# cmhungsteve/TA3N

Measured on AMD Instinct MI355X. Metric: src+tgt videos/sec per train step, UCF->HMDB_full 5-seg TA3N, higher is better.
Workload: dtype bf16

## Files before the change

ta3n_amd/csrc/ta3n_gemm_kernel.h:

```cpp
#pragma once
#include <hip/hip_runtime.h>
#include <cstdlib>
#include <cstring>

#include <type_traits>

#include "ta3n_kernels.h"

using namespace ta3n;

namespace {

typedef float f32x16 __attribute__((ext_vector_type(16)));
typedef __attribute__((address_space(3))) void lds_void_t;

constexpr int BKC = 64;

__device__ __forceinline__ float4 zero4() { return make_float4(0.f, 0.f, 0.f, 0.f); }

__device__ __forceinline__ void glds16(const float *gsrc, unsigned lds_byte_addr) {
    unsigned keep;
    lds_byte_addr = __builtin_amdgcn_readfirstlane(lds_byte_addr);
    asm volatile("s_mov_b32 %0, m0\n\ts_mov_b32 m0, %2\n\ts_nop 0\n\tglobal_load_lds_dwordx4 %1, off\n\ts_mov_b32 m0, %0"
                 : "=&s"(keep) : "v"(gsrc), "s"(lds_byte_addr) : "memory");
// ... 37 lines not shown
    asm volatile("s_mov_b32 %0, m0\n\ts_mov_b32 m0, %2\n\ts_nop 0\n\tglobal_load_lds_dword %1, off\n\ts_mov_b32 m0, %0"
                 : "=&s"(keep) : "v"(gsrc), "s"(lds_byte_addr) : "memory");
}

template <int R, int NW>
__device__ __attribute__((noinline)) void issue_slow(const float *__restrict__ origin, int ld, int kmajor, int r0, int rvalid, int k0,
                                                     int krem, unsigned lds_addr, int wave, int lane, const float *__restrict__ zeros) {
#pragma unroll 1
    for (int q = wave; q < R; q += NW) {
        const float *src;
        if (!kmajor) {
            const int k = 4 * ((lane >> 2) ^ (q & 15)) + (lane & 3);
            src = (r0 + q < rvalid && k < krem) ? origin + (size_t)(r0 + q) * ld + k0 + k : zeros;
        } else {
            constexpr int KPP = 64 / R;
            const int k = q * KPP + lane / R;
            const int r = r0 + lane % R;
            src = (r < rvalid && k < krem) ? origin + (size_t)(k0 + k) * ld + r : zeros;
        }
        glds4(src, lds_addr + q * 256);
    }
}

constexpr int K_NEVER = 1 << 28;

template <int R, int NW, bool TW = false, bool PAIR = false, bool HS = false>
struct OperandStream {
    static constexpr int NP = HS ? R / 8 / NW : R / 4 / NW;
    static_assert(HS ? (R / 8) % NW == 0 && TW && !PAIR : (R / 4) % NW == 0, "pieces must divide over the waves");
    const float *p[NP];
    int kofs[NP];
    int step;
    const float *origin;
    int ld, kmajor, r0, rvalid;
    bool vec;

    __device__ __forceinline__ void setup(const float *__restrict__ origin_, int ld_, int kmajor_, int klen, int r0_, int rvalid_,
                                          int wave, int lane, int pair_delta = 0) {
        origin = origin_; ld = ld_; kmajor = kmajor_; r0 = r0_; rvalid = rvalid_;
        if constexpr (TW && PAIR) {
            vec = true;
            const int ldf = ld_ >> 1;
            step = kmajor_ ? 64 * ldf : BKC / 2;
#pragma unroll
            for (int i = 0; i < NP; ++i) {
                const int q = wave + NW * i;
// ... 17 lines not shown
            vec = true;
            const int ldf = ld_ >> 1;
            step = kmajor_ ? 64 * ldf : BKC / 2;
#pragma unroll
            for (int i = 0; i < NP; ++i) {
                const int q = wave + NW * i;
                if (!kmajor_) {
                    const int row = q * 8 + (lane >> 3);
                    const int slot = (lane & 7) ^ ((row >> 1) & 7);
                    p[i] = origin_ + (size_t)(r0_ + row) * ldf + 4 * slot;
                    kofs[i] = (r0_ + row < rvalid_) ? 8 * slot : K_NEVER;
                } else {
                    constexpr int LPR = R / 8, KPP = 64 / LPR;
                    const int k = q * KPP + lane / LPR;
                    const int chunk = (lane % LPR) ^ (R == 64 ? ((k >> 1) & 1) << 2 : R == 128 ? (k & 3) << 2 : 0);
                    const int r = r0_ + chunk * 8;
                    p[i] = origin_ + (size_t)k * ldf + (r >> 1);
                    kofs[i] = (r < rvalid_) ? k : K_NEVER;
                }
            }
            return;
        }
        if constexpr (TW) {
            vec = true;
            const int ldf = ld_ >> 1;
            step = kmajor_ ? 128 * ldf : BKC;
#pragma unroll
            for (int i = 0; i < NP; ++i) {
                const int q = wave + NW * i;
                if (!kmajor_) {
                    const int row = q * 4 + (lane >> 4);
                    const int slot = (lane & 15) ^ (row & 15);
                    p[i] = origin_ + (size_t)(r0_ + row) * ldf + 4 * slot;
                    kofs[i] = (r0_ + row < rvalid_) ? 8 * slot : K_NEVER;
                } else {
                    constexpr int LPR = R / 8, KPP = 64 / LPR;
                    const int k = q * KPP + lane / LPR;
                    const int chunk = (lane % LPR) ^ (R == 64 ? ((k >> 1) & 1) << 2 : R == 128 ? (k & 3) << 2 : 0);
                    const int r = r0_ + chunk * 8;
                    p[i] = origin_ + (size_t)k * ldf + (r >> 1);
                    kofs[i] = (r < rvalid_) ? k : K_NEVER;
                }
            }
            return;
        }
        const int off_bits = (int)(reinterpret_cast<uintptr_t>(origin_) >> 2);
        vec = kmajor_ ? (((off_bits | ld_ | r0_ | rvalid_) & 3) == 0) : (((off_bits | ld_ | klen) & 3) == 0);
// ... 6 lines not shown
                const int row = q * 4 + (lane >> 4);
                const int k = 4 * ((lane & 15) ^ (row & 15));
                p[i] = origin_ + (size_t)(r0_ + row) * ld_ + k;
                kofs[i] = (r0_ + row < rvalid_) ? k : K_NEVER;
            } else {
                constexpr int LPR = R / 4, KPP = 64 / LPR;
                const int k = q * KPP + lane / LPR;
                const int r = r0_ + (lane % LPR) * 4;
                p[i] = origin_ + (size_t)k * ld_ + r;
                kofs[i] = (r < rvalid_) ? k : K_NEVER;
            }
        }
    }

    __device__ __forceinline__ void issue(int k0, int krem, unsigned lds_addr, int wave, int lane, const float *__restrict__ zeros) {
        if (vec) {
            const float *src[NP];
#pragma unroll
            for (int i = 0; i < NP; ++i) {
                src[i] = kofs[i] < krem ? p[i] : zeros;
                p[i] += step;
            }
            glds16_batch<NP>(src, lds_addr + wave * 1024, NW * 1024);
        } else {
            issue_slow<R, NW>(origin, ld, kmajor, r0, rvalid, k0, krem, lds_addr, wave, lane, zeros);
        }
    }
};

typedef short s16x4 __attribute__((ext_vector_type(4)));
typedef float f32x4 __attribute__((ext_vector_type(4)));
typedef __bf16 bf16x2 __attribute__((ext_vector_type(2)));
typedef __bf16 bf16x8 __attribute__((ext_vector_type(8)));
typedef float f32x2 __attribute__((ext_vector_type(2)));
typedef unsigned u32x2 __attribute__((ext_vector_type(2)));
typedef unsigned u32x4 __attribute__((ext_vector_type(4)));


template <int BM, int BN, int WK, bool AKM, bool BKM, bool FULL, bool RS, int BF, int RM = 1, int RN = 1>
__device__ __forceinline__ void compute_stage(f32x16 (&accs)[RM][RN], float (&rss)[RM], const float *__restrict__ sa,
                                              const float *__restrict__ sb, int ra, int rb, int wk, int lh, int krem) {
    constexpr bool HS = BF == 5;
    constexpr int GPW = (HS ? 8 : 16) / WK;
    constexpr int NQ = GPW / 2;
    constexpr int ROWF = HS ? BKC / 2 : BKC;
    static_assert(GPW >= 2, "the K split leaves every wave a pair of k groups");
// ... 1078 lines not shown
```

ta3n_amd/csrc/ta3n_heads.hip:

```cpp
#include <hip/hip_runtime.h>

#include <mutex>

#include "../../include/ta3n_hip.h"
#include "ta3n_kernels.h"

using namespace ta3n;

namespace {

typedef float f32x4 __attribute__((ext_vector_type(4)));


constexpr int NBH = 256;
constexpr int RPW = HEADS_RPW;
constexpr int WROW = 68;
constexpr int TROW = 260;

template <int VPW>
struct Lds {
    static_assert(VPW == 1 || VPW == 2, "1 or 2 videos per workgroup");
    static constexpr int W = 0;
    static constexpr int VD = W + NBH * WROW;
    static constexpr int HV = VD + VPW * NBH;
    static constexpr int GHV = HV + VPW * NBH;
    static constexpr int GVT = GHV + VPW * NBH;
    static constexpr int GY = GVT + VPW * NBH;
    static constexpr int PR = GY + VPW * 64;
    static constexpr int GPV = PR + VPW * 128;
    static constexpr int Y = GPV + 8;
    static constexpr int FPART = Y + VPW * 64;
    static constexpr int VPART = FPART + 16 * NBH;
    static constexpr int LOSS = VPART + 4 * NBH;
    static constexpr int TOTAL = LOSS + 32;
    static constexpr int WPV = 4 / VPW;
};
static_assert(64 * TROW <= NBH * WROW, "backward tile / classifier staging must fit in the weight tile");
constexpr int S_LOSS_MIN = Lds<1>::LOSS;

#ifdef TA3N_HEADS_TIMING
#define STAMP(i) do { if ((int)blockIdx.x == g.n_frm_wg + 100 && threadIdx.x == 0) { reinterpret_cast<unsigned long long *>(ptrs.ws + g.o_gattn)[i] = __builtin_amdgcn_s_memtime(); } } while (0)
#else
#define STAMP(i) do { } while (0)
#endif

__device__ __forceinline__ bool video_valid(int Bs, int valid_source, int valid_target, int b) {
    return b < Bs ? (b < valid_source) : (b - Bs < valid_target);
}

struct StepScalars {
    int valid_source, valid_target;
    float inv_n_cls, inv_n_rel, inv_n_vid, inv_n_frm, inv_n_ent, gamma, beta1, p_drop_v;
    uint32_t seed_v;
};
__device__ __forceinline__ StepScalars step_scalars(const Hyper *__restrict__ hy) {
    StepScalars h;
    h.valid_source = hy->valid_source; h.valid_target = hy->valid_target;
    h.inv_n_cls = hy->inv_n_cls; h.inv_n_rel = hy->inv_n_rel; h.inv_n_vid = hy->inv_n_vid; h.inv_n_frm = hy->inv_n_frm;
    h.inv_n_ent = hy->inv_n_ent; h.gamma = hy->gamma; h.beta1 = hy->beta[1]; h.p_drop_v = hy->p_drop_v; h.seed_v = hy->seed_v;
    return h;
}

__device__ __forceinline__ void write_loss_part(float *smem, float *ws, int o_loss_part, int wg, float gamma, int S_LOSS) {
    const int tid = threadIdx.x;
    __syncthreads();
    float v = 0.f;
    if (tid < 8) v = (smem[S_LOSS + tid] + smem[S_LOSS + 8 + tid]) + (smem[S_LOSS + 16 + tid] + smem[S_LOSS + 24 + tid]);
    __syncthreads();
// ... 5 lines not shown
    }
}

template <int VPW, bool PIPE>
__device__ __forceinline__ void video_wg(const Geom g, const Ptrs ptrs, float *smem) {
    using L = Lds<VPW>;
    constexpr int S_W = L::W, S_VD = L::VD, S_HV = L::HV, S_GHV = L::GHV, S_GVT = L::GVT, S_GY = L::GY, S_PR = L::PR, S_GPV = L::GPV, S_Y = L::Y,
                  S_FPART = L::FPART, S_VPART = L::VPART, S_LOSS = L::LOSS, WPV = L::WPV;
    float *__restrict__ ws = ptrs.ws;
    const float *__restrict__ wsr = ptrs.ws;
    const float *__restrict__ P = ptrs.p;
    const Hyper *__restrict__ hy = reinterpret_cast<const Hyper *>(ptrs.ws + g.o_hyper);
    const int *__restrict__ tf = reinterpret_cast<const int *>(ptrs.ws + g.o_tuple_first);
    const int *__restrict__ labels = reinterpret_cast<const int *>(ptrs.ws + g.o_labels);
    const int tid = threadIdx.x, lane = tid & 63, wv = tid >> 6;
    const int NR = g.n_rel, NT = g.n_tuples, C = g.C;
    const int b0 = ((int)blockIdx.x - g.n_frm_wg) * VPW;
    const int nv = min(VPW, g.B - b0);
    const int vloc = wv / WPV, sub = wv % WPV;
    const int b = b0 + vloc;
    const bool have = vloc < nv;
    const bool lead = sub == 0;
    const bool attn_on = (g.flags & TA3N_FLAG_TRANS_ATTN) != 0;
    const bool train = hy->train != 0;
    const StepScalars hs = step_scalars(hy);
    const float inv_keep_v = hyper_scale(hy, SK_INV_KEEP_V);
    const bool drop_v = train && hs.p_drop_v > 0.f;
    const float *__restrict__ Wdv = P + g.p_Wdv;
    const float *__restrict__ Wcv = P + g.p_Wcv;
    float l_cls = 0.f, l_rel = 0.f, l_vid = 0.f, l_ent = 0.f;

    const int tfv = lane <= NR ? tf[lane] : 0;
    struct RelIn { float hr[4], w0[4], w1[4], zr[3][4], b0, b1; int nt; };
    auto load_rel = [&](int j, RelIn &o) {
        const float *__restrict__ W2f = P + g.p_W2_0 + (size_t)j * g.p_W2_stride;
        const float *__restrict__ hrf = wsr + g.o_Hr + ((size_t)b * NR + j) * NBH;
        const int ju = __builtin_amdgcn_readfirstlane(j);
        const int t_lo = __builtin_amdgcn_readlane(tfv, ju);
        const int t_hi = __builtin_amdgcn_readlane(tfv, ju + 1);
        o.nt = t_hi - t_lo;
#pragma unroll
        for (int q = 0; q < 4; ++q) { o.hr[q] = hrf[q * 64 + lane]; o.w0[q] = W2f[q * 64 + lane]; o.w1[q] = W2f[NBH + q * 64 + lane]; }
#pragma unroll
        for (int tt = 0; tt < 3; ++tt) {
            const bool on = tt < o.nt;
#pragma unroll
// ... 35 lines not shown
#pragma unroll 1
            for (int j = sub; j < NR; j += WPV) {
                RelIn rel_nxt = rel_cur;
                if (PIPE && j + WPV < NR) load_rel(j + WPV, rel_nxt);
                float d0 = 0.f, d1 = 0.f;
                float r[4] = {0.f, 0.f, 0.f, 0.f};
#pragma unroll
                for (int q = 0; q < 4; ++q) {
                    d0 = fmaf(rel_cur.hr[q], rel_cur.w0[q], d0);
                    d1 = fmaf(rel_cur.hr[q], rel_cur.w1[q], d1);
                }
#pragma unroll
                for (int tt = 0; tt < 3; ++tt)
#pragma unroll
                    for (int q = 0; q < 4; ++q) r[q] += rel_cur.zr[tt][q];
                d0 = wave_allreduce_sum(d0) + rel_cur.b0;
                d1 = wave_allreduce_sum(d1) + rel_cur.b1;
                if (PIPE) rel_cur = rel_nxt;
                float w = 0.f;
                if (attn_on) w = 1.f - soft2(d0, d1).H;
#pragma unroll
                for (int q = 0; q < 4; ++q) {
                    ws[g.o_R + ((size_t)b * NR + j) * NBH + q * 64 + lane] = r[q];
                    vacc[q] += attn_on ? (w + 1.f) * r[q] : r[q];
                }
                if (lane == 0) {
                    ws[g.o_Pr + ((size_t)b * NR + j) * 2 + 0] = d0;
                    ws[g.o_Pr + ((size_t)b * NR + j) * 2 + 1] = d1;
                    ws[g.o_attn + (size_t)b * NR + j] = attn_on ? w : r[0];
                    smem[S_PR + (vloc * 64 + j) * 2 + 0] = d0;
                    smem[S_PR + (vloc * 64 + j) * 2 + 1] = d1;
                }
            }
        }
#pragma unroll
        for (int q = 0; q < 4; ++q) smem[S_VPART + wv * NBH + q * 64 + lane] = vacc[q];
    }
    __syncthreads();
#pragma unroll
    for (int v = 0; v < VPW; ++v) {
        float val = 0.f;
#pragma unroll
        for (int s_ = 0; s_ < WPV; ++s_) val += smem[S_VPART + (v * WPV + s_) * NBH + tid];
        float vd = val;
        if (drop_v) vd = val * keep_mask(hs.seed_v, (uint32_t)((b0 + v) * NBH + tid), hs.p_drop_v) * inv_keep_v;
        if (v < nv) {
            ws[g.o_V + (size_t)(b0 + v) * NBH + tid] = val;
            ws[g.o_Vd + (size_t)(b0 + v) * NBH + tid] = vd;
        }
        smem[S_VD + v * NBH + tid] = v < nv ? vd : 0.f;
    }
    STAMP(1);
#pragma unroll
    for (int i = 0; i < 16; ++i) {
        const int f = i * 256 + tid;
        if (f < C * 64) *reinterpret_cast<f32x4 *>(&smem[S_W + (f >> 6) * TROW + (f & 63) * 4]) = cw[i];
    }
    __syncthreads();

    STAMP(2);
    {
        const int c = tid >> 2, part = tid & 3;
#pragma unroll
        for (int v = 0; v < VPW; ++v) {
            float acc = 0.f;
            if (c < C) {
                const float *wr = &smem[S_W + c * TROW + part * 64];
                const float *vd = &smem[S_VD + v * NBH + part * 64];
#pragma unroll
                for (int k4 = 0; k4 < 64; k4 += 4) {
                    const float4 w4 = *reinterpret_cast<const float4 *>(wr + k4);
// ... 19 lines not shown
        const int n = srow + 16 * c16;
#pragma unroll
        for (int v = 0; v < VPW; ++v) {
            f32x4 xk[4];
#pragma unroll
            for (int kc = 0; kc < 4; ++kc) xk[kc] = *reinterpret_cast<const f32x4 *>(&smem[S_VD + v * NBH + kc * 64 + sk4]);
            float hv = 0.f;
#pragma unroll
            for (int i = 0; i < 16; ++i) {
                float p = 0.f;
#pragma unroll
                for (int kc = 0; kc < 4; ++kc) {
                    const f32x4 w4 = wreg[kc * 16 + i];
                    p = fmaf(w4.x, xk[kc].x, p); p = fmaf(w4.y, xk[kc].y, p); p = fmaf(w4.z, xk[kc].z, p); p = fmaf(w4.w, xk[kc].w, p);
                }
                p += dpp_move<0xB1, 0xF>(0.f, p);
                p += dpp_move<0x4E, 0xF>(0.f, p);
                p += dpp_move<0x141, 0xF>(0.f, p);
                p += dpp_move<0x140, 0xF>(0.f, p);
                if (c16 == i) hv = p;
            }
            const float h = fmaxf(hv + bdv_n, 0.f);
            smem[S_HV + v * NBH + n] = h;
            if (v < nv) ws[g.o_Hv + (size_t)(b0 + v) * NBH + n] = h;
        }
    }
    __syncthreads();

    STAMP(4);
    {
        float d0 = 0.f, d1 = 0.f;
#pragma unroll
        for (int q = 0; q < 4; ++q) {
            const float h = smem[S_HV + vloc * NBH + q * 64 + lane];
            d0 = fmaf(h, wc0[q], d0);
            d1 = fmaf(h, wc1[q], d1);
        }
        d0 = wave_allreduce_sum(d0) + bcdv0;
        d1 = wave_allreduce_sum(d1) + bcdv1;
        const float m = wave_allreduce_max(y);
        const float e = lane < C ? expf(y - m) : 0.f;
        const float ls = logf(wave_allreduce_sum(e));
        const float lp = lane < C ? y - m - ls : 0.f;
        const float pr = lane < C ? expf(lp) : 0.f;
        const float Hc = wave_allreduce_sum(-pr * lp);
        float gy = 0.f, g0 = 0.f, g1 = 0.f;
        if (have && lead) {
// ... 3 lines not shown
            const Soft2 s = soft2(d0, d1);
            const bool ent_on = (g.flags & TA3N_FLAG_ATTN_ENTROPY) && valid;
            const float ce = hs.gamma * hs.inv_n_ent;
            if (cls_on) {
                gy = (pr - (lane == label ? 1.f : 0.f)) * hs.inv_n_cls;
                if (lane == label) l_cls = -lp * hs.inv_n_cls;
            }
            if (ent_on) {
                gy += ce * (1.f + s.H) * (-pr * (lp + Hc));
                if (lane == 0) l_ent = (1.f + s.H) * Hc * hs.inv_n_ent;
            }
            if (lane >= C) gy = 0.f;
            if ((g.flags & TA3N_FLAG_ADV_VIDEO) && valid) {
                const int d = is_src ? 0 : 1;
                if (lane == 0) l_vid = -(d ? s.lp1 : s.lp0) * hs.inv_n_vid;
                g0 = (s.p0 - (d == 0 ? 1.f : 0.f)) * hs.inv_n_vid;
                g1 = (s.p1 - (d == 1 ? 1.f : 0.f)) * hs.inv_n_vid;
            }
            if (ent_on) {
                g0 += ce * Hc * (-s.p0 * (s.lp0 + s.H));
                g1 += ce * Hc * (-s.p1 * (s.lp1 + s.H));
            }
            if (lane < C) ws[g.o_gY + (size_t)b * C + lane] = gy;
            if (lane == 0) {
                ws[g.o_Pv + (size_t)b * 2] = d0; ws[g.o_Pv + (size_t)b * 2 + 1] = d1;
                ws[g.o_gPv + (size_t)b * 2] = g0; ws[g.o_gPv + (size_t)b * 2 + 1] = g1;
            }
        }
        if (lead) {
            smem[S_GY + vloc * 64 + lane] = gy;
            if (lane == 0) { smem[S_GPV + vloc * 2] = g0; smem[S_GPV + vloc * 2 + 1] = g1; }
        }
        l_cls = wave_allreduce_sum(l_cls);
    }
    __syncthreads();

    STAMP(5);
#pragma unroll
    for (int v = 0; v < VPW; ++v) {
        const float gh = smem[S_HV + v * NBH + tid] > 0.f ? smem[S_GPV + v * 2] * wct0 + smem[S_GPV + v * 2 + 1] * wct1 : 0.f;
        smem[S_GHV + v * NBH + tid] = gh;
        if (v < nv) ws[g.o_gHv + (size_t)(b0 + v) * NBH + tid] = gh;
    }
    __syncthreads();

    struct RelBack { float w20[4], w21[4], hrv[4], rv[4]; };
    auto load_back = [&](int j, RelBack &o) {
        const size_t bj = (size_t)b * NR + j;
        const float *__restrict__ W2 = P + g.p_W2_0 + (size_t)j * g.p_W2_stride;
#pragma unroll
        for (int q = 0; q < 4; ++q) {
            const int c = q * 64 + lane;
            o.w20[q] = W2[c]; o.w21[q] = W2[NBH + c];
            o.hrv[q] = wsr[g.o_Hr + bj * NBH + c];
            o.rv[q] = ws[g.o_R + bj * NBH + c];
        }
    };
    RelBack back_cur;
#pragma unroll
    for (int q = 0; q < 4; ++q) back_cur.w20[q] = back_cur.w21[q] = back_cur.hrv[q] = back_cur.rv[q] = 0.f;
    if (PIPE && have && sub < NR) load_back(sub, back_cur);

#pragma unroll
    for (int v = 0; v < VPW; ++v) {
        float gh[16];
// ... 42 lines not shown
#pragma unroll
            for (int q = 0; q < 4; ++q) { w20[q] = back_cur.w20[q]; w21[q] = back_cur.w21[q]; hrv[q] = back_cur.hrv[q]; rv[q] = back_cur.rv[q]; }
            if (PIPE) back_cur = back_nxt;
            const float z0 = smem[S_PR + (vloc * 64 + j) * 2], z1 = smem[S_PR + (vloc * 64 + j) * 2 + 1];
            const Soft2 s = soft2(z0, z1);
            float g0 = 0.f, g1 = 0.f;
            if (adv_rel) {
                const int d = is_src ? 0 : 1;
                if (lane == 0) l_rel += -(d ? s.lp1 : s.lp0) * hs.inv_n_rel;
                g0 = (s.p0 - (d == 0 ? 1.f : 0.f)) * hs.inv_n_rel;
                g1 = (s.p1 - (d == 1 ? 1.f : 0.f)) * hs.inv_n_rel;
            }
            if (lane == 0) { ws[g.o_gPr + bj * 2] = g0; ws[g.o_gPr + bj * 2 + 1] = g1; }
            float w1 = 1.f;
            if (attn_on) {
                float dot = 0.f;
#pragma unroll
                for (int q = 0; q < 4; ++q) dot = fmaf(rv[q], gv[q], dot);
                dot = wave_allreduce_sum(dot);
                g0 += dot * s.p0 * (s.lp0 + s.H);
                g1 += dot * s.p1 * (s.lp1 + s.H);
                w1 = 1.f + (1.f - s.H);
            }
            if (lane == 0) { ws[g.o_gPrT + bj * 2] = g0; ws[g.o_gPrT + bj * 2 + 1] = g1; }
#pragma unroll
            for (int q = 0; q < 4; ++q) {
                const int c = q * 64 + lane;
                ws[g.o_gRa + bj * NBH + c] = w1 * gv[q];
                ws[g.o_gHr + bj * NBH + c] = hrv[q] > 0.f ? g0 * w20[q] + g1 * w21[q] : 0.f;
            }
        }
    }
    {
        auto lane0 = [](float x) { return __builtin_bit_cast(float, __builtin_amdgcn_readlane(__builtin_bit_cast(int, x), 0)); };
        const float lr = lane0(l_rel), lv = lane0(l_vid), le = lane0(l_ent);
        if (lane < 8) {
            float v = 0.f;
            if (lane == 1) v = l_cls;
            if (lane == 2) v = lr;
            if (lane == 3) v = lv;
            if (lane == 5) v = le;
            smem[S_LOSS + wv * 8 + lane] = v;
        }
    }
    STAMP(7);
    write_loss_part(smem, ws, g.o_loss_part, (int)blockIdx.x - g.n_frm_wg, hs.gamma, S_LOSS);
    STAMP(8);
}

template <int FQ>
__device__ __forceinline__ void frame_wg(const Geom g, const Ptrs ptrs, float *smem, int wg) {
    float *__restrict__ ws = ptrs.ws;
// ... 148 lines not shown
```

ta3n_amd/csrc/ta3n_plan.cpp:

```cpp
#include "ta3n_plan.h"
#include "ta3n_kernels.h"

#include <algorithm>
#include <cstdlib>
#include <cstring>
#include <sstream>

using namespace ta3n;

int64_t ta3n_plan::poff(const std::string &name) const {
    for (const auto &p : params)
        if (p.name == name) return p.off;
    return -1;
}
int64_t ta3n_plan::woff(const std::string &name) const {
    for (const auto &r : regions)
        if (r.name == name) return r.off;
    return -1;
}

namespace {

int64_t align_up(int64_t v, int64_t a) { return (v + a - 1) / a * a; }

// ... 548 lines not shown
        for (int i = ph.task_begin; i < ph.task_begin + ph.task_count; ++i) {
            const Task &t = p.tasks[i];
            if (t.seg_count == 0) continue;
            if (t.c_base == BASE_WS) produced.push_back({t.c_off, t.c_off + (int64_t)(t.m_valid - 1) * t.c_ld + t.n_valid});
            for (int f = 0; f < t.fan_count; ++f)
                produced.push_back({t.fan_out_off[f], t.fan_out_off[f] + (int64_t)(t.m_valid - 1) * t.fan_ld + t.n_valid});
        }
    }
    std::vector<Span> read16;
    for (Phase &ph : p.phases) {
        if (!in_family(ph.group) || ph.kind != PH_GEMM) continue;
        bool ok = true;
        std::vector<Span> reads;
        std::vector<char> seen(p.segs.size(), 0);
        for (int i = ph.task_begin; i < ph.task_begin + ph.task_count && ok; ++i) {
            const Task &t = p.tasks[i];
            for (int k = t.seg_begin; k < t.seg_begin + t.seg_count && ok; ++k) {
                if (seen[k]) continue;
                seen[k] = 1;
                const Seg &sg = p.segs[k];
                const int a_rows = sg.pad[0] > 0 ? sg.pad[0] : t.m_valid, b_rows = t.n_valid;
                auto side_ok = [&](int base, int off, int ld, int kmajor, int rows) {
                    if (base == BASE_G) return false;
                    if (((off | ld) & 7) != 0) return false;
                    if ((kmajor ? rows : sg.klen) & 7) return false;
                    if (base == BASE_WS) {
                        const Span rd = kmajor ? Span{off, off + (int64_t)(sg.klen - 1) * ld + rows}
                                               : Span{off, off + (int64_t)(rows - 1) * ld + sg.klen};
                        bool covered = false;
                        for (auto &pr : produced) covered = covered || overlaps(rd, pr);
                        if (!covered) return false;
                        reads.push_back(rd);
                    }
                    return true;
                };
                ok = side_ok(sg.a_base, sg.a_off, sg.a_ld, sg.a_kmajor, a_rows) &&
                     side_ok(sg.b_base, sg.b_off, sg.b_ld, sg.b_kmajor, b_rows);
            }
        }
        if (!ok) continue;
        ph.bf16 |= 16;
        read16.insert(read16.end(), reads.begin(), reads.end());
        std::fill(seen.begin(), seen.end(), 0);
        for (int i = ph.task_begin; i < ph.task_begin + ph.task_count; ++i) {
            const Task &t = p.tasks[i];
            for (int k = t.seg_begin; k < t.seg_begin + t.seg_count; ++k) {
                if (seen[k]) continue;
                seen[k] = 1;
// ... 576 lines not shown
    g.o_gHf = (int32_t)b.add_region("gHf", (int64_t)BT * F);
    g.o_gVt = (int32_t)b.add_region("gVt", (int64_t)B * NB);
    g.o_gPrT = (int32_t)b.add_region("gPrT", (int64_t)B * NR * 2);
    g.o_gRa = (int32_t)b.add_region("gRa", (int64_t)B * NR * NB);
    g.o_gHr = (int32_t)b.add_region("gHr", (int64_t)B * NR * NB);
    g.o_gR = (int32_t)b.add_region("gR", (int64_t)B * NR * NB);
    g.o_gZ = (int32_t)b.add_region("gZ", (int64_t)B * NT * NB);
    g.o_gZ1 = (int32_t)b.add_region("gZ1", (int64_t)BT * F);
    SharedStack st;
    lay_out_stack(p, b, st, BT, F, g.o_F1, g.o_gZ1);
    if (feat_grads) g.o_gV_ext = (int32_t)b.add_region("gV_ext", (int64_t)B * NB);
    if (bn_shared) {
        g.o_Z0 = (int32_t)b.add_region("Z0", (int64_t)BT * F);
        g.o_gZ0 = (int32_t)b.add_region("gZ0", (int64_t)BT * F);
        g.o_bn_batch = (int32_t)b.add_region("bn_batch", (int64_t)2 * 3 * F);
        g.o_bn_run = (int32_t)b.add_region("bn_run", (int64_t)2 * 2 * F);
        g.p_bn_w[0] = (int32_t)P("bn_shared_S.weight"); g.p_bn_b[0] = (int32_t)P("bn_shared_S.bias");
        g.p_bn_w[1] = (int32_t)P("bn_shared_T.weight"); g.p_bn_b[1] = (int32_t)P("bn_shared_T.bias");
    }
    if (mcd) {
        g.o_Y2 = (int32_t)b.add_region("Y2", (int64_t)B * C);
        g.o_gY2 = (int32_t)b.add_region("gY2", (int64_t)B * C);
    }
#ifdef TA3N_GEMM_STAMPS
    b.add_region("stamps", 8192 * 16 * 2);
#endif
    g.o_zeros = (int32_t)b.add_region("zeros", 64);
    g.o_ones = (int32_t)b.add_region("ones", (int64_t)BT * 4);
    if (g.o_ones != g.o_zeros + 64) { err = "internal: ones must follow zeros"; return TA3N_ERR_INVALID; }
    g.o_losses = (int32_t)b.add_region("losses", 8);
    g.n_norm_blocks = 256;
    g.o_norm_part = (int32_t)b.add_region("norm_part", g.n_norm_blocks);
    g.o_grad_norm = (int32_t)b.add_region("grad_norm", 4);
    g.o_hyper = (int32_t)b.add_region("hyper", 32);
    g.o_labels = (int32_t)b.add_region("labels", B);
    g.o_tuple_first = (int32_t)b.add_region("tuple_first", NR + 1);
    g.heads_vpw = B > 224 ? 2 : 1;
    if (const char *e = std::getenv("TA3N_HEADS_VPW")) { const int v = std::atoi(e); if (v == 1 || v == 2) g.heads_vpw = v; }
    g.n_vid_wg = (B + g.heads_vpw - 1) / g.heads_vpw;
    g.heads_rpw = HEADS_RPW;
    while (g.n_vid_wg + (BT + g.heads_rpw - 1) / g.heads_rpw > 256 && g.heads_rpw < 8 * HEADS_RPW) g.heads_rpw *= 2;
    g.n_frm_wg = (BT + g.heads_rpw - 1) / g.heads_rpw;
    g.o_fh_part = (int32_t)b.add_region("fh_part", (int64_t)g.n_frm_wg * 2 * F);
    g.o_fh_bpart = (int32_t)b.add_region("fh_bpart", (int64_t)g.n_frm_wg * 2);
    g.o_loss_part = (int32_t)b.add_region("loss_part", (int64_t)(g.n_vid_wg + g.n_frm_wg) * 8);
    g.o_metrics = (int32_t)b.add_region("metrics", 8);
// ... 167 lines not shown
            s.push_back(spec_gR(j));
            s.push_back(wgrad(NB, NB, B, g.o_gHr + (int64_t)j * NB, ldR, g.o_R + (int64_t)j * NB, ldR, W1(j), B1(j)));
            s.push_back(wgrad(2, NB, B, g.o_gPrT + (int64_t)j * 2, NR * 2, g.o_Hr + (int64_t)j * NB, ldR, W2(j), B2(j)));
        }
    };
    auto push_trn_wgrads = [&](std::vector<GemmSpec> &s, unsigned scale_mask = ~0u) {
        for (int j = 0; j < NR; ++j) {
            if (!((scale_mask >> (j & 31)) & 1)) continue;
            const int sl = T - j;
            for (int pos = 0; pos < sl; ++pos) {
                GemmSpec gw;
                gw.M = NB; gw.N = F;
                gw.affinity = 100 + j;
                for (int t = p.tuple_first[j]; t < p.tuple_first[j + 1]; ++t)
                    gw.segs.push_back(mkseg(KM(BASE_WS, g.o_gZ + (int64_t)t * NB, ldZ),
                                            KM(BASE_WS, g.o_F1 + (int64_t)tau(t, pos) * F, ldF), B));
                gw.proto = proto(BASE_G, trnW(j) + (int64_t)pos * F, sl * F);
                if (pos == 0) { gw.proto.epi |= EPI_ROWSUM_A; gw.proto.bias_base = BASE_G; gw.proto.bias_off = (int32_t)trnB(j); }
                s.push_back(gw);
            }
        }
    };
    int split_f1_grad = 0;
    auto push_f1_grad = [&](std::vector<GemmSpec> &s) {
        for (int f = 0; f < T; ++f) {
            GemmSpec gz;
            gz.M = B; gz.N = F;
            gz.affinity = 200 + f;
            gz.segs.push_back(mkseg(KC(BASE_WS, g.o_gHf + (int64_t)f * F, ldF), KM(BASE_P, Wfd, F), F, SK_NEG_BETA_FRM));
            for (int t = 0; t < NT; ++t) {
                const int j = p.scale_id[t], sl = p.scale_len[t];
                for (int pos = 0; pos < sl; ++pos)
                    if (tau(t, pos) == f)
                        gz.segs.push_back(mkseg(KC(BASE_WS, g.o_gZ + (int64_t)t * NB, ldZ),
                                                KM(BASE_P, trnW(j) + (int64_t)pos * F, sl * F), NB));
            }
            gz.proto = proto(BASE_WS, g.o_gZ1 + (int64_t)f * F, ldF);
            with_mask(gz.proto, g.o_F1 + (int64_t)f * F, ldF);
            gz.proto.gamma_kind = SK_INV_KEEP_I;
            gz.split = split_f1_grad;
            s.push_back(gz);
        }
    };
    auto push_trn_level = [&](std::vector<GemmSpec> &s) { push_trn_wgrads(s); push_f1_grad(s); };
    auto push_shared_fc_wgrad = [&](std::vector<GemmSpec> &s) {
        GemmSpec gw;
        gw.M = F; gw.N = D;
        gw.segs.push_back(mkseg(KM(BASE_WS, bn_shared ? g.o_gZ0 : st.o_gZ[1], F), KM(BASE_X, 0, D), BT));
        gw.proto = proto(BASE_G, Wsh, D);
        gw.proto.epi |= EPI_ROWSUM_A; gw.proto.bias_base = BASE_G; gw.proto.bias_off = (int32_t)bsh;
        s.push_back(gw);
    };

    { std::vector<GemmSpec> s{spec_F1()}; b.add_gemm_phase(0, s); }
    if (bn_shared) b.add_simple_phase(PH_BN_FWD, 0);
    add_stack_forward(b, st, 0, BT, F);
    {
        std::vector<GemmSpec> s{spec_Hf()};
        for (int t = 0; t < NT; ++t) s.push_back(spec_Z(t));
        b.add_gemm_phase(0, s);
    }
// ... 7 lines not shown
    { std::vector<GemmSpec> s{spec_Y(), spec_Hv()}; if (mcd) s.push_back(spec_Y2()); b.add_gemm_phase(0, s); }
    { std::vector<GemmSpec> s{spec_Pv()}; b.add_gemm_phase(0, s); }
    b.add_simple_phase(PH_LOSS, 1);
    {
        std::vector<GemmSpec> s{spec_gHv(), spec_gHf()};
        push_video_head_wgrads(s);
        s.push_back(wgrad(2, F, BT, g.o_gPf, 2, g.o_Hf, F, Wcd, bcd));
        b.add_gemm_phase(2, s);
    }
    {
        std::vector<GemmSpec> s{spec_gVt()};
        push_video_disc_wgrads(s);
        push_frame_disc_wgrads(s);
        b.add_gemm_phase(2, s);
    }
    b.add_simple_phase(PH_POOL_BWD, 2);
    { std::vector<GemmSpec> s; push_relation_level(s); b.add_gemm_phase(2, s); }
    { std::vector<GemmSpec> s; push_trn_level(s); b.add_gemm_phase(2, s); }
    add_stack_backward(b, st, 2, BT, F);
    if (bn_shared) b.add_simple_phase(PH_BN_BWD, 2);
    { std::vector<GemmSpec> s; push_shared_fc_wgrad(s); b.add_gemm_phase(2, s); }
    b.add_simple_phase(PH_GRAD_NORM, 3);
    b.add_simple_phase(PH_SGD, 3);
    if (heads_supported(NB, C, F) && !mcd && !feat_grads && !(bn_shared && c.chain != 0)) {
        const bool chain = c.chain != 0;
        std::string cerr;
        auto forward_levels = [&](int group, const std::vector<Task> *side) {
            if (chain) b.begin_chain();
            { std::vector<GemmSpec> s{spec_F1()}; b.add_gemm_phase(group, s); }
            if (side) {
                if (chain) b.chain_append(*side);
                else { for (auto &t : *side) p.tasks.push_back(t); p.phases.back().task_count += (int32_t)side->size(); }
            }
            if (!chain && group == 5) return;
            if (bn_shared) b.add_simple_phase(PH_BN_FWD, group);
            add_stack_forward(b, st, group, BT, F);
            {
                std::vector<GemmSpec> s{spec_Hf()};
                for (int t = 0; t < NT; ++t) s.push_back(spec_Z(t));
                b.add_gemm_phase(group, s);
            }
            {
                std::vector<GemmSpec> s;
                for (int j = 0; j < NR; ++j) s.push_back(spec_Hr(j));
                b.add_gemm_phase(group, s);
            }
            if (chain) { const std::string e = b.end_chain(); if (!e.empty()) cerr = e; }
        };
        split_shared_fc = ((c.split_k & 4) && !chain && !bn_shared) ? 1 : 0;
        forward_levels(4, nullptr);
        b.add_simple_phase(PH_HEADS, 4);
        b.sum8[0] = g.o_losses; b.sum8[1] = g.o_loss_part; b.sum8[2] = g.n_vid_wg + g.n_frm_wg;
        {
            std::vector<GemmSpec> s;
            push_relation_level(s);
            push_video_head_wgrads(s);
            push_video_disc_wgrads(s);
            b.colsum_pending(g.o_fh_part, g.n_frm_wg, 2 * F, 2 * F, Wcd);
            b.colsum_pending(g.o_fh_bpart, g.n_frm_wg, 2, 2, bcd);
            const bool twins = (c.flags & (TA3N_FLAG_BF16_MFMA | TA3N_FLAG_F32_SPLIT)) && (c.flags & TA3N_FLAG_BF16_STORE);
            if (!twins) push_frame_disc_wgrads(s);
            b.add_gemm_phase(4, s);
        }
        const bool twins_on = (c.flags & (TA3N_FLAG_BF16_MFMA | TA3N_FLAG_F32_SPLIT)) && (c.flags & TA3N_FLAG_BF16_STORE);
        const unsigned late_mask = c.wgrads_late == 0 ? 0u : c.wgrads_late == 1 ? ~0u : (unsigned)c.wgrads_late;
        const bool late_fd = (late_mask >> 1) & 1;
        const unsigned late_trn = late_mask >> 2;
        if (chain) b.begin_chain();
        split_f1_grad = ((c.split_k & 2) && !chain) ? 2 : 0;
        {
            std::vector<GemmSpec> s;
            if (chain) {
                push_f1_grad(s);
                if (twins_on && !late_fd) push_frame_disc_wgrads(s);
                push_trn_wgrads(s, ~late_trn);
            } else {
                if (twins_on && !late_fd) push_frame_disc_wgrads(s);
                push_trn_wgrads(s, ~late_trn);
                push_f1_grad(s);
            }
            b.add_gemm_phase(4, s);
        }
        add_stack_backward(b, st, 4, BT, F);
        if (bn_shared) b.add_simple_phase(PH_BN_BWD, 4);
        {
            std::vector<GemmSpec> s;
            push_shared_fc_wgrad(s);
            push_trn_wgrads(s, late_trn);
            if (twins_on && late_fd) push_frame_disc_wgrads(s);
            b.add_gemm_phase(4, s);
        }
        if (chain) { const std::string e = b.end_chain(); if (!e.empty()) cerr = e; }
        {
            const Phase *f1 = nullptr;
            for (const Phase &ph : p.phases)
                if (ph.group == 4 && ph.kind == PH_GEMM) { f1 = &ph; break; }
            b.force_next = f1->wm * 100 + f1->wn * 10 + f1->wk + 1000 * ((f1->bf16 & 15) + ((f1->bf16 & 64) ? 3 : 0)) +
                           10000 * blk_code(f1->rm, f1->rn);
            const int64_t i0 = p.first_floats / 4, i1 = p.live_floats / 4;
            const int n_side = 256;
// ... 5 lines not shown
                t.epi = EPI_SGD;
                t.sig = -1;
                t.c_base = BASE_NONE; t.bias_base = BASE_NONE; t.aux_base = BASE_NONE; t.add_base = BASE_NONE;
                t.pad[0] = (int32_t)std::min(i0 + per * k, i1);
                t.pad[1] = (int32_t)std::min(i0 + per * (k + 1), i1);
                side.push_back(t);
            }
            forward_levels(5, &side);
        }
        if (!cerr.empty()) { err = cerr; return TA3N_ERR_INVALID; }
        std::vector<size_t> grad_tasks;
        for (const Phase &ph : p.phases)
            if (ph.group == 4 && ph.kind == PH_GEMM)
                for (int i = ph.task_begin; i < ph.task_begin + ph.task_count; ++i)
                    if ((p.tasks[i].seg_count > 0 || (p.tasks[i].epi & EPI_COLSUM)) && p.tasks[i].c_base == BASE_G) grad_tasks.push_back((size_t)i);
        const int n_bn_slots = bn_shared ? 2 * ((F + BN_COLS - 1) / BN_COLS) : 0;
        g.n_sumsq = (int32_t)grad_tasks.size() + n_bn_slots;
        g.o_sumsq = (int32_t)b.add_region("sumsq", g.n_sumsq);
        for (size_t k = 0; k < grad_tasks.size(); ++k) {
            p.tasks[grad_tasks[k]].epi |= EPI_SUMSQ;
            p.tasks[grad_tasks[k]].pad[3] = g.o_sumsq + (int32_t)k;
        }
        std::vector<Span> kept{Span{g.o_gHf, g.o_gHf + (int64_t)BT * F}};
        std::vector<Span> gemm_only{Span{g.o_gZ, g.o_gZ + (int64_t)B * NT * NB}};
        if (bn_shared) {
            kept.push_back(Span{g.o_F1, g.o_F1 + (int64_t)BT * F});
            kept.push_back(Span{g.o_gZ0, g.o_gZ0 + (int64_t)BT * F});
        } else {
            gemm_only.push_back(Span{g.o_gZ1, g.o_gZ1 + (int64_t)BT * F});
            for (int k = 1; k < st.L; ++k) gemm_only.push_back(Span{st.o_gZ[k], st.o_gZ[k] + (int64_t)BT * F});
        }
        add_bf16_twins(p, b, g, BT, D, kept, gemm_only);
        if (p.ws_floats >= (1ll << 31)) { err = "workspace too large for 32-bit offsets"; return TA3N_ERR_INVALID; }
    } else {
        add_bf16_twins(p, b, g, BT, D, {}, {});
        if (p.ws_floats >= (1ll << 31)) { err = "workspace too large for 32-bit offsets"; return TA3N_ERR_INVALID; }
    }
    if (b.mixed_kinds) { err = "internal: a GEMM spec mixes operand kinds across its K segments"; return TA3N_ERR_INVALID; }
    if (b.n_split_pairs > 0) {
        std::vector<int64_t> pair_off(b.n_split_pairs, -1);
        int64_t floats = 0;
        for (const Phase &ph : p.phases) {
            if (ph.kind != PH_GEMM) continue;
            const int64_t tile = (int64_t)(32 * ph.wm * std::max(ph.rm, 1)) * (32 * ph.wn * std::max(ph.rn, 1));
            for (int i = ph.task_begin; i < ph.task_begin + ph.task_count; ++i) {
                const Task &t = p.tasks[i];
                if ((t.epi & EPI_SPLITK) && pair_off[t.pad[0]] < 0) { pair_off[t.pad[0]] = floats; floats += 2 * tile; }
            }
        }
        const int64_t o_part = b.add_region("splitk_part", floats);
        const int64_t o_tick = b.add_region("splitk_ticket", b.n_split_pairs);
        for (auto &t : p.tasks)
            if (t.epi & EPI_SPLITK) {
                const int pair = t.pad[0];
                t.pad[0] = (int32_t)(o_part + pair_off[pair]);
                t.pad[1] = (int32_t)(o_tick + pair);
            }
        if (p.ws_floats >= (1ll << 31)) { err = "workspace too large for 32-bit offsets"; return TA3N_ERR_INVALID; }
    }
    for (auto &t : p.tasks)
        if (t.seg_count > 0) t.seg0 = p.segs[t.seg_begin];
    return TA3N_OK;
}

int ta3n::build_plan(ta3n_plan &p, std::string &err) {
    const ta3n_config cfg = p.cfg;
    uint64_t deny = 0;
    for (int attempt = 0; attempt < 16; ++attempt) {
        p = ta3n_plan();
        p.cfg = cfg;
        p.deny_blocking = deny;
        const int rc = build_plan_once(p, err);
        if (rc != TA3N_OK) return rc;
        uint64_t bad = 0;
        for (size_t i = 0; i < p.phases.size(); ++i) {
            const Phase &ph = p.phases[i];
            if (ph.kind == PH_GEMM && (ph.rm * ph.rn > 1 || (ph.bf16 & 64)) && !(ph.bf16 & 16)) bad |= 1ull << (i & 63);
        }
        if (bad == 0) return TA3N_OK;
        deny |= bad;
    }
    err = "internal: register-blocked tile selection did not settle";
    return TA3N_ERR_INVALID;
}
```

ta3n_amd/csrc/ta3n_plan.h:

```cpp
#pragma once
#include <string>
#include <vector>

#include "../../include/ta3n_hip.h"
#include "ta3n_types.h"

struct ParamInfo {
    std::string name;
    int64_t off;
    int32_t rows, cols;
    bool live;
};

struct Region {
    std::string name;
    int64_t off, size;
};

struct ta3n_plan {
    ta3n_config cfg;
    ta3n::Geom geom;
    std::vector<ParamInfo> params;
    int64_t param_floats = 0, live_floats = 0;
    int64_t first_floats = 0;
    std::vector<Region> regions;
    int64_t ws_floats = 0;
    int64_t ws_floats_before_twins = 0;
    std::vector<ta3n::Seg> segs;
    std::vector<ta3n::Task> tasks;
    std::vector<ta3n::Phase> phases;
    std::vector<ta3n::Wait> waits;
    std::vector<int32_t> tuples, scale_len, scale_id, tuple_first;
    int n_tuples = 0;
    std::vector<int32_t> phase_kinds;
    uint64_t deny_blocking = 0;
    void *d_segs = nullptr;
    void *d_tasks = nullptr;
    void *d_waits = nullptr;
    bool uploaded = false;
    int device = -1;

    int64_t poff(const std::string &name) const;
    int64_t woff(const std::string &name) const;
};

namespace ta3n {
int build_plan(ta3n_plan &p, std::string &err);
void set_error(const std::string &msg);
}
```

Baseline: 1.964 million.

## Host frame-disc input-grad GEMM in relation phase with bf16 twins for heads outputs

Moves the frame-discriminator input-gradient GEMM (gHf·Wfd) into the relation GEMM phase, writing to a new gF1fd buffer. The F1 gradient GEMMs then add that buffer instead of recomputing the segment, which shortens the critical F1-grad phase and fills the relation phase. To keep that phase in bf16, the heads kernel now writes bf16 twin copies of R, Vd, Hv, gHv, gY, gPv, gPrT and gHr. The operand loader gains a narrow k-major twin path for odd-aligned operands. The plan builder retries with hosting disabled if the relation phase falls off the twin path. Costs are extra workspace, extra twin stores in the heads kernel, and added plan complexity.

```diff
diff --git a/ta3n_amd/csrc/ta3n_gemm_kernel.h b/ta3n_amd/csrc/ta3n_gemm_kernel.h
--- a/ta3n_amd/csrc/ta3n_gemm_kernel.h
+++ b/ta3n_amd/csrc/ta3n_gemm_kernel.h
@@ -83,6 +83,22 @@
     }
 }
 
+template <int R, int NW>
+__device__ __attribute__((noinline)) void issue_slow_twin(const float *__restrict__ origin, int ld, int r0, int rvalid, int k0, int krem,
+                                                          unsigned lds_addr, int wave, int lane, const float *__restrict__ zeros) {
+    constexpr int DPR = R / 2, KPP = 64 / DPR;
+    static_assert(R == 32 || R == 64 || R == 128, "k-major twin images exist for 32-, 64- and 128-row operands");
+#pragma unroll 1
+    for (int q = wave; q < R; q += NW) {
+        const int k = q * KPP + lane / DPR;
+        const int pd = lane % DPR;
+        const int chunk = (pd >> 2) ^ (R == 64 ? ((k >> 1) & 1) << 2 : R == 128 ? (k & 3) << 2 : 0);
+        const int r = r0 + 8 * chunk + 2 * (pd & 3);
+        const float *src = (r < rvalid && k < krem) ? origin + (((size_t)(k0 + k) * ld + r) >> 1) : zeros;
+        glds4(src, lds_addr + q * 256);
+    }
+}
+
 constexpr int K_NEVER = 1 << 28;
 
 template <int R, int NW, bool TW = false, bool PAIR = false, bool HS = false>
@@ -146,7 +162,8 @@
             return;
         }
         if constexpr (TW) {
-            vec = true;
+            vec = !(kmajor_ && ((ld_ | rvalid_) & 7) != 0);
+            if (!vec) return;
             const int ldf = ld_ >> 1;
             step = kmajor_ ? 128 * ldf : BKC;
 #pragma unroll
@@ -199,6 +216,8 @@
                 p[i] += step;
             }
             glds16_batch<NP>(src, lds_addr + wave * 1024, NW * 1024);
+        } else if constexpr (TW) {
+            if constexpr (!PAIR && !HS) issue_slow_twin<R, NW>(origin, ld, r0, rvalid, k0, krem, lds_addr, wave, lane, zeros);
         } else {
             issue_slow<R, NW>(origin, ld, kmajor, r0, rvalid, k0, krem, lds_addr, wave, lane, zeros);
         }
diff --git a/ta3n_amd/csrc/ta3n_heads.hip b/ta3n_amd/csrc/ta3n_heads.hip
--- a/ta3n_amd/csrc/ta3n_heads.hip
+++ b/ta3n_amd/csrc/ta3n_heads.hip
@@ -44,6 +44,10 @@
 #define STAMP(i) do { } while (0)
 #endif
 
+__device__ __forceinline__ void store_twin(float *ws, const Geom &g, size_t e, float v) {
+    reinterpret_cast<unsigned short *>(ws + g.o_ws16)[e] = (unsigned short)pack_bf16(v, 0.f);
+}
+
 __device__ __forceinline__ bool video_valid(int Bs, int valid_source, int valid_target, int b) {
     return b < Bs ? (b < valid_source) : (b - Bs < valid_target);
 }
@@ -95,6 +99,7 @@
     const bool have = vloc < nv;
     const bool lead = sub == 0;
     const bool attn_on = (g.flags & TA3N_FLAG_TRANS_ATTN) != 0;
+    const bool tw = g.o_ws16 >= 0 && g.pair_delta == 0;
     const bool train = hy->train != 0;
     const StepScalars hs = step_scalars(hy);
     const float inv_keep_v = hyper_scale(hy, SK_INV_KEEP_V);
@@ -176,6 +181,7 @@
 #pragma unroll
                 for (int q = 0; q < 4; ++q) {
                     ws[g.o_R + ((size_t)b * NR + j) * NBH + q * 64 + lane] = r[q];
+                    if (tw) store_twin(ws, g, g.o_R + ((size_t)b * NR + j) * NBH + q * 64 + lane, r[q]);
                     vacc[q] += attn_on ? (w + 1.f) * r[q] : r[q];
                 }
                 if (lane == 0) {
@@ -201,6 +207,7 @@
         if (v < nv) {
             ws[g.o_V + (size_t)(b0 + v) * NBH + tid] = val;
             ws[g.o_Vd + (size_t)(b0 + v) * NBH + tid] = vd;
+            if (tw) store_twin(ws, g, g.o_Vd + (size_t)(b0 + v) * NBH + tid, vd);
         }
         smem[S_VD + v * NBH + tid] = v < nv ? vd : 0.f;
     }
@@ -266,7 +273,10 @@
             }
             const float h = fmaxf(hv + bdv_n, 0.f);
             smem[S_HV + v * NBH + n] = h;
-            if (v < nv) ws[g.o_Hv + (size_t)(b0 + v) * NBH + n] = h;
+            if (v < nv) {
+                ws[g.o_Hv + (size_t)(b0 + v) * NBH + n] = h;
+                if (tw) store_twin(ws, g, g.o_Hv + (size_t)(b0 + v) * NBH + n, h);
+            }
         }
     }
     __syncthreads();
@@ -316,9 +326,11 @@
                 g1 += ce * Hc * (-s.p1 * (s.lp1 + s.H));
             }
             if (lane < C) ws[g.o_gY + (size_t)b * C + lane] = gy;
+            if (tw && lane < C) store_twin(ws, g, g.o_gY + (size_t)b * C + lane, gy);
             if (lane == 0) {
                 ws[g.o_Pv + (size_t)b * 2] = d0; ws[g.o_Pv + (size_t)b * 2 + 1] = d1;
                 ws[g.o_gPv + (size_t)b * 2] = g0; ws[g.o_gPv + (size_t)b * 2 + 1] = g1;
+                if (tw) { store_twin(ws, g, g.o_gPv + (size_t)b * 2, g0); store_twin(ws, g, g.o_gPv + (size_t)b * 2 + 1, g1); }
             }
         }
         if (lead) {
@@ -334,7 +346,10 @@
     for (int v = 0; v < VPW; ++v) {
         const float gh = smem[S_HV + v * NBH + tid] > 0.f ? smem[S_GPV + v * 2] * wct0 + smem[S_GPV + v * 2 + 1] * wct1 : 0.f;
         smem[S_GHV + v * NBH + tid] = gh;
-        if (v < nv) ws[g.o_gHv + (size_t)(b0 + v) * NBH + tid] = gh;
+        if (v < nv) {
+            ws[g.o_gHv + (size_t)(b0 + v) * NBH + tid] = gh;
+            if (tw) store_twin(ws, g, g.o_gHv + (size_t)(b0 + v) * NBH + tid, gh);
+        }
     }
     __syncthreads();
 
@@ -423,12 +438,17 @@
                 g1 += dot * s.p1 * (s.lp1 + s.H);
                 w1 = 1.f + (1.f - s.H);
             }
-            if (lane == 0) { ws[g.o_gPrT + bj * 2] = g0; ws[g.o_gPrT + bj * 2 + 1] = g1; }
+            if (lane == 0) {
+                ws[g.o_gPrT + bj * 2] = g0; ws[g.o_gPrT + bj * 2 + 1] = g1;
+                if (tw) { store_twin(ws, g, g.o_gPrT + bj * 2, g0); store_twin(ws, g, g.o_gPrT + bj * 2 + 1, g1); }
+            }
 #pragma unroll
             for (int q = 0; q < 4; ++q) {
                 const int c = q * 64 + lane;
                 ws[g.o_gRa + bj * NBH + c] = w1 * gv[q];
-                ws[g.o_gHr + bj * NBH + c] = hrv[q] > 0.f ? g0 * w20[q] + g1 * w21[q] : 0.f;
+                const float ghr = hrv[q] > 0.f ? g0 * w20[q] + g1 * w21[q] : 0.f;
+                ws[g.o_gHr + bj * NBH + c] = ghr;
+                if (tw) store_twin(ws, g, g.o_gHr + bj * NBH + c, ghr);
             }
         }
     }
diff --git a/ta3n_amd/csrc/ta3n_plan.cpp b/ta3n_amd/csrc/ta3n_plan.cpp
--- a/ta3n_amd/csrc/ta3n_plan.cpp
+++ b/ta3n_amd/csrc/ta3n_plan.cpp
@@ -594,8 +594,9 @@
                 const int a_rows = sg.pad[0] > 0 ? sg.pad[0] : t.m_valid, b_rows = t.n_valid;
                 auto side_ok = [&](int base, int off, int ld, int kmajor, int rows) {
                     if (base == BASE_G) return false;
-                    if (((off | ld) & 7) != 0) return false;
-                    if ((kmajor ? rows : sg.klen) & 7) return false;
+                    const bool wide = ((off | ld) & 7) == 0 && ((kmajor ? rows : sg.klen) & 7) == 0;
+                    const bool narrow = kmajor && base == BASE_WS && ((off | ld) & 1) == 0 && !(c.flags & TA3N_FLAG_F32_SPLIT) && !(ph.bf16 & 64);
+                    if (!wide && !narrow) return false;
                     if (base == BASE_WS) {
                         const Span rd = kmajor ? Span{off, off + (int64_t)(sg.klen - 1) * ld + rows}
                                                : Span{off, off + (int64_t)(rows - 1) * ld + sg.klen};
@@ -1218,6 +1219,11 @@
         g.o_Y2 = (int32_t)b.add_region("Y2", (int64_t)B * C);
         g.o_gY2 = (int32_t)b.add_region("gY2", (int64_t)B * C);
     }
+    const bool fused_step = heads_supported(NB, C, F) && !mcd && !feat_grads && !(bn_shared && c.chain != 0);
+    const bool plain_twins = (c.flags & TA3N_FLAG_BF16_MFMA) && (c.flags & TA3N_FLAG_BF16_STORE);
+    const bool host_fd = fused_step && plain_twins && live_frm && B > 128 && c.chain == 0 && !(c.split_k & (2 | 8)) && !p.relation_host_denied;
+    const int64_t o_gF1fd = host_fd ? b.add_region("gF1fd", (int64_t)BT * F) : -1;
+    p.relation_hosts_fd = host_fd;
 #ifdef TA3N_GEMM_STAMPS
     b.add_region("stamps", 8192 * 16 * 2);
 #endif
@@ -1431,12 +1437,20 @@
         }
     };
     int split_f1_grad = 0;
+    bool f1_add_fd = false;
+    auto spec_gF1fd = [&]() {
+        GemmSpec gf;
+        gf.M = BT; gf.N = F;
+        gf.segs.push_back(mkseg(KC(BASE_WS, g.o_gHf, F), KM(BASE_P, Wfd, F), F, SK_NEG_BETA_FRM));
+        gf.proto = proto(BASE_WS, o_gF1fd, F);
+        return gf;
+    };
     auto push_f1_grad = [&](std::vector<GemmSpec> &s) {
         for (int f = 0; f < T; ++f) {
             GemmSpec gz;
             gz.M = B; gz.N = F;
             gz.affinity = 200 + f;
-            gz.segs.push_back(mkseg(KC(BASE_WS, g.o_gHf + (int64_t)f * F, ldF), KM(BASE_P, Wfd, F), F, SK_NEG_BETA_FRM));
+            if (!f1_add_fd) gz.segs.push_back(mkseg(KC(BASE_WS, g.o_gHf + (int64_t)f * F, ldF), KM(BASE_P, Wfd, F), F, SK_NEG_BETA_FRM));
             for (int t = 0; t < NT; ++t) {
                 const int j = p.scale_id[t], sl = p.scale_len[t];
                 for (int pos = 0; pos < sl; ++pos)
@@ -1446,6 +1460,7 @@
             }
             gz.proto = proto(BASE_WS, g.o_gZ1 + (int64_t)f * F, ldF);
             with_mask(gz.proto, g.o_F1 + (int64_t)f * F, ldF);
+            if (f1_add_fd) with_add(gz.proto, o_gF1fd + (int64_t)f * F, ldF);
             gz.proto.gamma_kind = SK_INV_KEEP_I;
             gz.split = split_f1_grad;
             s.push_back(gz);
@@ -1499,7 +1514,7 @@
     { std::vector<GemmSpec> s; push_shared_fc_wgrad(s); b.add_gemm_phase(2, s); }
     b.add_simple_phase(PH_GRAD_NORM, 3);
     b.add_simple_phase(PH_SGD, 3);
-    if (heads_supported(NB, C, F) && !mcd && !feat_grads && !(bn_shared && c.chain != 0)) {
+    if (fused_step) {
         const bool chain = c.chain != 0;
         std::string cerr;
         auto forward_levels = [&](int group, const std::vector<Task> *side) {
@@ -1537,6 +1552,11 @@
             b.colsum_pending(g.o_fh_bpart, g.n_frm_wg, 2, 2, bcd);
             const bool twins = (c.flags & (TA3N_FLAG_BF16_MFMA | TA3N_FLAG_F32_SPLIT)) && (c.flags & TA3N_FLAG_BF16_STORE);
             if (!twins) push_frame_disc_wgrads(s);
+            if (host_fd) {
+                if (!(c.wgrads_late == 1 || (c.wgrads_late > 1 && ((c.wgrads_late >> 1) & 1)))) push_frame_disc_wgrads(s);
+                s.push_back(spec_gF1fd());
+            }
+            p.relation_phase = (int)p.phases.size();
             b.add_gemm_phase(4, s);
         }
         const bool twins_on = (c.flags & (TA3N_FLAG_BF16_MFMA | TA3N_FLAG_F32_SPLIT)) && (c.flags & TA3N_FLAG_BF16_STORE);
@@ -1545,6 +1565,7 @@
         const unsigned late_trn = late_mask >> 2;
         if (chain) b.begin_chain();
         split_f1_grad = ((c.split_k & 2) && !chain) ? 2 : 0;
+        f1_add_fd = host_fd;
         {
             std::vector<GemmSpec> s;
             if (chain) {
@@ -1552,7 +1573,7 @@
                 if (twins_on && !late_fd) push_frame_disc_wgrads(s);
                 push_trn_wgrads(s, ~late_trn);
             } else {
-                if (twins_on && !late_fd) push_frame_disc_wgrads(s);
+                if (twins_on && !late_fd && !host_fd) push_frame_disc_wgrads(s);
                 push_trn_wgrads(s, ~late_trn);
                 push_f1_grad(s);
             }
@@ -1604,6 +1625,13 @@
             p.tasks[grad_tasks[k]].pad[3] = g.o_sumsq + (int32_t)k;
         }
         std::vector<Span> kept{Span{g.o_gHf, g.o_gHf + (int64_t)BT * F}};
+        if (host_fd) {
+            for (int32_t o : {g.o_R, g.o_gHr}) kept.push_back(Span{o, o + (int64_t)B * NR * NB});
+            for (int32_t o : {g.o_Vd, g.o_Hv, g.o_gHv}) kept.push_back(Span{o, o + (int64_t)B * NB});
+            kept.push_back(Span{g.o_gY, g.o_gY + (int64_t)B * C});
+            kept.push_back(Span{g.o_gPv, g.o_gPv + (int64_t)B * 2});
+            kept.push_back(Span{g.o_gPrT, g.o_gPrT + (int64_t)B * NR * 2});
+        }
         std::vector<Span> gemm_only{Span{g.o_gZ, g.o_gZ + (int64_t)B * NT * NB}};
         if (bn_shared) {
             kept.push_back(Span{g.o_F1, g.o_F1 + (int64_t)BT * F});
@@ -1648,10 +1676,12 @@
 int ta3n::build_plan(ta3n_plan &p, std::string &err) {
     const ta3n_config cfg = p.cfg;
     uint64_t deny = 0;
+    bool deny_host = false;
     for (int attempt = 0; attempt < 16; ++attempt) {
         p = ta3n_plan();
         p.cfg = cfg;
         p.deny_blocking = deny;
+        p.relation_host_denied = deny_host;
         const int rc = build_plan_once(p, err);
         if (rc != TA3N_OK) return rc;
         uint64_t bad = 0;
@@ -1659,6 +1689,8 @@
             const Phase &ph = p.phases[i];
             if (ph.kind == PH_GEMM && (ph.rm * ph.rn > 1 || (ph.bf16 & 64)) && !(ph.bf16 & 16)) bad |= 1ull << (i & 63);
         }
+        const bool host_off_twins = bad == 0 && p.relation_hosts_fd && p.relation_phase >= 0 && !(p.phases[p.relation_phase].bf16 & 16);
+        if (host_off_twins) { deny_host = true; continue; }
         if (bad == 0) return TA3N_OK;
         deny |= bad;
     }
diff --git a/ta3n_amd/csrc/ta3n_plan.h b/ta3n_amd/csrc/ta3n_plan.h
--- a/ta3n_amd/csrc/ta3n_plan.h
+++ b/ta3n_amd/csrc/ta3n_plan.h
@@ -33,6 +33,8 @@
     std::vector<int32_t> tuples, scale_len, scale_id, tuple_first;
     int n_tuples = 0;
     std::vector<int32_t> phase_kinds;
+    int relation_phase = -1;
+    bool relation_hosts_fd = false, relation_host_denied = false;
     uint64_t deny_blocking = 0;
     void *d_segs = nullptr;
     void *d_tasks = nullptr;
```

Result: slower. 1.883 million (-4.2%).
